# ariel415el/SoundEventDetection-Pytorch

Measured on AMD Instinct MI355X. Metric: SED train clips/sec (60s,64-mel,9-layer CNN), higher is better.
Workload: dtype bf16; 1 GPU; Cnn_AvgPooling main widths [32, 64, 128, 128], 60 s / 32 kHz / 64-mel clips (T=6001 frames, NFFT 1024, hop 320), batch 32/GPU, train step = waveform->log-mel->fwd->BCE->bwd->Adam-amsgrad; frontend_constants=bench, graph_replay=False, global_batch=32, frames=6001, parallelism=dp1, frontend_in_step=True, frontend_overlapped=False, frontend_overlap_mode=0, sync_bn=False, rccl_group=False, collectives_executed=False

## Files before the change

soundeventdetection-pytorch_amd/csrc/sed_conv_pc.hip:

```cpp
#include "conv_common.h"

#include <stdlib.h>


namespace {

#ifdef SED_STAMPS
constexpr bool kStamps = true;
#else
constexpr bool kStamps = false;
#endif

constexpr int kPcBlocks = 256;

__device__ __forceinline__ void wg_barrier() {
    asm volatile("s_waitcnt lgkmcnt(0)\n\ts_barrier" ::: "memory");
}

__device__ __forceinline__ int xswz(int col) { return (col >> 2) & 3; }
__device__ __forceinline__ f32x16 zero16() {
    f32x16 z;
#pragma unroll
    for (int i = 0; i < 16; ++i) z[i] = 0.f;
    return z;
}


template <typename T, int W, int WP, int TH, bool WRITE_MASK>
__device__ __forceinline__ void c1_build_tail(const C1Mma& c1m, const f32x16& d, T* __restrict__ xsb, int bi, int lane, int b, int h0, int H,
                                              unsigned short* __restrict__ maskg) {
    const int rr = bi >> 1, half = bi & 1, hh = lane >> 5;
    const int hr = h0 - 1 + rr;
    const int coll = half * 32 + (lane & 31) + 1;
    T* dst = xsb + (rr * WP + coll) * 32 + hh * 4;
    const int sw = (coll >> 2) & 3;
    if (hr < 0 || hr >= H) {
        asm volatile("" ::: "memory");
        float z4[4] = {0.f, 0.f, 0.f, 0.f};
#pragma unroll
        for (int g4 = 0; g4 < 4; ++g4) store4<T>(dst + ((g4 ^ sw) * 8), z4);
        return;
    }
    unsigned mk;
    const bool wm = WRITE_MASK && maskg != nullptr && (rr >= 2 || (rr == 1 && h0 == 0));
#if !defined(SED_C1_PKTAIL) || SED_C1_PKTAIL
    unsigned w[8];
    if (wm) c1mma_block_tail_pk<true>(d, w, mk);
    else c1mma_block_tail_pk<false>(d, w, mk);
#pragma unroll
    for (int g4 = 0; g4 < 4; ++g4) {
        u32x2 v2 = {w[2 * g4], w[2 * g4 + 1]};
        *reinterpret_cast<u32x2*>(dst + ((g4 ^ sw) * 8)) = v2;
    }
#else
    float a[16];
    if (wm) c1mma_block_tail<true>(c1m, d, a, mk);
    else c1mma_block_tail<false>(c1m, d, a, mk);
#pragma unroll
    for (int g4 = 0; g4 < 4; ++g4) {
// ... 19 lines not shown
#define DIV_TPI(n) ((n) / p.tilesPerImg)
#define DIV_NCH(n) ((n) / nchunks)
#endif
#ifndef SED_PC_ZEROC
#define SED_PC_ZEROC 0
#endif
#ifndef SED_PC_ONECH
#define SED_PC_ONECH 1
#endif
#ifndef SED_PC_WREGS
#define SED_PC_WREGS 1
#endif
#ifndef SED_PC_CSTAT
#define SED_PC_CSTAT 0
#endif
template <int W, int BN, int PRO, int EPI, bool COL = false, int NPW = 4, bool BLD = false, bool WR = false>
__global__ __launch_bounds__(256 + 64 * NPW + (BLD ? 256 : 0)) void conv_pc_kernel(ConvParams p) {
    typedef bf16_t T;
    constexpr int BM = 256, TH = BM / W, ROWS = TH + 2, WP = (W + 2 + 3) & ~3;
    constexpr int XS = ROWS * WP * 32;
    constexpr int WS = WR ? 0 : 9 * 32 * BN;
    constexpr int NT = BN / 32;
    constexpr int BNP = BN + 8;
    constexpr int OSZ = BM * BNP;
    constexpr int NP = 64 * NPW;
    constexpr int NTHR = 256 + NP + (BLD ? 256 : 0);
    static_assert(!WR || (!COL && !BLD && PRO != SED_PRO_C1 && EPI != SED_EPI_RELUBWD_C1 && (BN == 64 || BN == 128)), "WR: plain layers, 64 / 128-channel slices");
    static_assert(!(PRO == SED_PRO_DZBN || PRO == SED_PRO_DZPOOL) || (!COL && !BLD && TH % 2 == 0), "dz on load: even tile heights (pooled rows)");
    static_assert(!BLD || PRO == SED_PRO_C1, "builder waves: C1 mode, the four waves after the loader waves");
    constexpr int XITEMS = ROWS * W * 4, XIPT = (XITEMS + NP - 1) / NP;
    constexpr int WITEMS = WS / 8, WIPT = WR ? 1 : (WITEMS + NP - 1) / NP;
    constexpr int IPR = BN / 8, FIPT = BM * IPR / NP, FQS = NP / IPR;
    static_assert(W >= 8 && BM % W == 0 && (BM * IPR) % NP == 0 && NP % IPR == 0, "geometry");
    constexpr bool C1PRO = PRO == SED_PRO_C1;
    constexpr bool DZPRO = PRO == SED_PRO_DZBN || PRO == SED_PRO_DZPOOL;
    constexpr int NCOEF = DZPRO ? 5 : 2;
    constexpr bool C1EPI = EPI == SED_EPI_RELUBWD_C1;
    constexpr bool RELUBWD = EPI == SED_EPI_RELUBWD || C1EPI;
    constexpr bool PSTATS = EPI == SED_EPI_POOLSTATS;
    static_assert(!(C1PRO || C1EPI) || W == 64, "C1 mode: a thread's items are consecutive rows of one column (W = 64)");
    static_assert(!C1EPI || BN == 32, "C1 epilogue: the output channels are conv1's 32");
    static_assert(!C1EPI || NPW == 4, "C1 epilogue: item u of a loader thread is tile row u (FQS = W)");

    extern __shared__ __attribute__((aligned(16))) char smem[];
    const int H = p.H, Cinp = p.Cinp, Coutp = p.Coutp;
    const int nchunks = Cinp >> 5;
// ... 6 lines not shown
    float* pcoef = reinterpret_cast<float*>(os + nos * OSZ);
    constexpr int XTW = W + 2, XTR = ROWS + 2, XTN = XTR * XTW;
    typedef C1Tile<W, XTR> XTL;
    bf16_t* xt0 = reinterpret_cast<bf16_t*>(pcoef + NCOEF * Cinp);

    const int tid = threadIdx.x, lane = tid & 63, wave = tid >> 6;
    const int NY = Coutp / BN;
    const unsigned logical = xcd_remap(blockIdx.x, gridDim.x);
    const int by = logical % NY, bx = logical / NY, nbx = gridDim.x / NY;
    const int n0 = by * BN;
    const T* __restrict__ wg = reinterpret_cast<const T*>(p.wpack);
    const size_t wchunk_bytes = (size_t)36 * Coutp * 8 * 2;

    const int t_begin = bx * p.tpb;
    const int t_end = min(p.totalTiles, t_begin + p.tpb);
    const int nst = (t_end > t_begin ? t_end - t_begin : 0) * nchunks;
    const int NI = (nst + (WR ? 3 : 2) + 1) & ~1;

    {
        constexpr int NPAD = 2 * ROWS * 2 * 4;
        bf16x8 z8;
#pragma unroll
        for (int e = 0; e < 8; ++e) z8[e] = (bf16_t)0.f;
        for (int i = tid; i < NPAD; i += NTHR) {
            const int c16 = i & 3, side = (i >> 2) & 1, rowi = (i >> 3) % ROWS, sg = (i >> 3) / ROWS;
            *reinterpret_cast<bf16x8*>(xs0 + sg * XS + (rowi * WP + (side ? W + 1 : 0)) * 32 + c16 * 8) = z8;
        }
    }
    if (PRO == SED_PRO_BNRELU || C1PRO) {
        for (int i = tid; i < 2 * Cinp; i += NTHR) pcoef[i] = (i < Cinp ? p.pro_scale[i] : p.pro_shift[i - Cinp]);
    }
// ... 2 lines not shown
        for (int i = tid; i < 5 * Cinp; i += NTHR) {
            const int rowc = i / Cinp, c = i - rowc * Cinp;
            float v = 0.f;
            if (rowc == 0) v = p.dz_ca[c] * inv_pool;
            else if (rowc == 1) v = p.dz_cb[c];
            else if (rowc == 2) v = p.dz_cc[c];
            else if (PRO == SED_PRO_DZPOOL) v = rowc == 3 ? p.dz_sc[c] : p.dz_sh[c];
            pcoef[i] = v;
        }
    }
    if constexpr (C1PRO) {
        c1tile_init<W, XTR>(xt0, tid, NTHR);
        c1tile_init<W, XTR>(xt0 + XTL::N, tid, NTHR);
        __syncthreads();
        if (nst > 0) {
            const int b = DIV_TPI(t_begin), h0 = (t_begin - b * p.tilesPerImg) * TH;
            for (int e = tid; e < XTN; e += NTHR) {
                const int r = e / XTW, c = e - r * XTW;
                const int hy = h0 - 2 + r, wx = c - 1;
                float v = 0.f;
                if (hy >= 0 && hy < H && wx >= 0 && wx < W) {
                    v = p.c1_x[((size_t)b * H + hy) * W + wx];
                    if (p.c1_mean) v = (v - p.c1_mean[wx]) * (1.0f / p.c1_std[wx]);
                }
                c1tile_store<W, XTR>(xt0, r, c, v);
            }
        }
    }
    if constexpr (!WR) if (wres && nst > 0) {
        const int total = nchunks * WITEMS;
        for (int i = tid; i < total; i += NTHR) {
            const int c = i / WITEMS, it = i - c * WITEMS;
            const int rowi = it / BN, off = (it - rowi * BN) * 8;
            *reinterpret_cast<bf16x8*>(ws + c * WS + it * 8) =
                *reinterpret_cast<const bf16x8*>(wg + ((size_t)(c * 36 + rowi) * Coutp + n0) * 8 + off);
        }
    }
    __syncthreads();

    float S[8], Q[8];
#pragma unroll
    for (int e = 0; e < 8; ++e) { S[e] = 0.f; Q[e] = 0.f; }

    C1Mma c1m;
// ... 3 lines not shown
    if (C1PRO && (C1SHARE || wave < 4 || wave >= 4 + NPW)) {
        c1mma_init(c1m, p.c1_w, p.pro_scale, p.pro_shift, lane);
        if constexpr (C1PRO) {
            c1tile_lane_offsets<W, XTR>(0, lane, c1o[0][0], c1o[0][1]);
            c1tile_lane_offsets<W, XTR>(1, lane, c1o[1][0], c1o[1][1]);
        }
    }
    auto c1mfma = [&](int js, int rr, int half) -> f32x16 {
        const bf16_t* row = xt0 + (js & 1) * XTL::N + rr * XTL::XP;
        return half ? c1mma_block_mfma_b(c1m, row, c1o[1][0], c1o[1][1]) : c1mma_block_mfma_b(c1m, row, c1o[0][0], c1o[0][1]);
    };
    unsigned short* __restrict__ maskg = reinterpret_cast<unsigned short*>(p.c1_mask);
    auto build_c1 = [&](int js, int bw, auto part_c) __attribute__((always_inline)) {
        constexpr int PART = decltype(part_c)::value;
        if (js >= nst || (SED_DBG(p, 4))) return;
        const int tile = t_begin + js;
        const int b = DIV_TPI(tile), h0 = (tile - b * p.tilesPerImg) * TH;
        static_assert(!C1PRO || ((2 * TH) % 4 == 0), "whole blocks per wave");
        constexpr int NB = (2 * TH) / 4;
        T* img = xs0 + (js & 1) * XS;
        const bool reuse = js > 0 && h0 > 0;
        static_assert(!C1PRO || NB == 2, "part 1 / part 2 = fresh-row blocks 0 / 1 of a wave");
        constexpr int B0 = PART == 2 ? 1 : 0, B1 = PART == 1 ? 1 : (PART == 3 ? 0 : NB);
        constexpr bool TOP = PART != 2 && PART != 4;
        f32x16 dd[NB + 1];
#pragma unroll
        for (int blk = B0; blk < B1; ++blk)
            dd[blk] = c1mfma(js, 2 + ((bw + 4 * blk) >> 1), (bw + 4 * blk) & 1);
        if (TOP && !reuse) dd[NB] = c1mfma(js, bw >> 1, bw & 1);
#pragma unroll
        for (int blk = B0; blk < B1; ++blk)
            c1_build_tail<T, W, WP, TH, EPI == SED_EPI_STATS>(c1m, dd[blk], img, 4 + bw + 4 * blk, lane, b, h0, H, maskg);
        if constexpr (!TOP) return;
        if (!reuse) {
            c1_build_tail<T, W, WP, TH, EPI == SED_EPI_STATS>(c1m, dd[NB], img, bw, lane, b, h0, H, maskg);
        } else {
            const T* prev = xs0 + ((js - 1) & 1) * XS + TH * WP * 32;
            constexpr int NIT = 2 * WP * 32 / 8;
#pragma unroll
            for (int it = 0; it < (NIT + 255) / 256; ++it) {
                const int q = bw * 64 + lane + 256 * it;
                if (q < NIT) *reinterpret_cast<bf16x8*>(img + q * 8) = *reinterpret_cast<const bf16x8*>(prev + q * 8);
            }
        }
    };

    constexpr int C1NB = (2 * TH) / 4, C1NCP = (2 * WP * 32 / 8 + 255) / 256;
    f32x16 bdd[C1PRO ? C1NB + 1 : 1];
    bf16x8 bcp[C1PRO ? C1NCP : 1];
    auto build_c1_issue = [&](int js, int bw) __attribute__((always_inline)) {
        if (js >= nst) return;
        const int tile = t_begin + js;
        const int b = DIV_TPI(tile), h0 = (tile - b * p.tilesPerImg) * TH;
        const bool reuse = js > 0 && h0 > 0;
#pragma unroll
        for (int blk = 0; blk < C1NB; ++blk)
            bdd[blk] = c1mfma(js, 2 + ((bw + 4 * blk) >> 1), (bw + 4 * blk) & 1);
        if (!reuse) {
            bdd[C1NB] = c1mfma(js, bw >> 1, bw & 1);
        } else {
            const T* prev = xs0 + ((js - 1) & 1) * XS + TH * WP * 32;
            constexpr int NIT = 2 * WP * 32 / 8;
#pragma unroll
            for (int it = 0; it < C1NCP; ++it) {
                const int q = bw * 64 + lane + 256 * it;
                if (q < NIT) bcp[it] = *reinterpret_cast<const bf16x8*>(prev + q * 8);
            }
        }
    };
    auto build_c1_finish = [&](int js, int bw) __attribute__((always_inline)) {
        if (js >= nst) return;
        const int tile = t_begin + js;
        const int b = DIV_TPI(tile), h0 = (tile - b * p.tilesPerImg) * TH;
        T* img = xs0 + (js & 1) * XS;
        const bool reuse = js > 0 && h0 > 0;
#pragma unroll
        for (int blk = 0; blk < C1NB; ++blk)
            c1_build_tail<T, W, WP, TH, EPI == SED_EPI_STATS>(c1m, bdd[blk], img, 4 + bw + 4 * blk, lane, b, h0, H, maskg);
        if (!reuse) {
            c1_build_tail<T, W, WP, TH, EPI == SED_EPI_STATS>(c1m, bdd[C1NB], img, bw, lane, b, h0, H, maskg);
        } else {
            constexpr int NIT = 2 * WP * 32 / 8;
#pragma unroll
            for (int it = 0; it < C1NCP; ++it) {
                const int q = bw * 64 + lane + 256 * it;
                if (q < NIT) *reinterpret_cast<bf16x8*>(img + q * 8) = bcp[it];
            }
        }
    };
#if !defined(SED_C1_SPLITBUILD)
#define SED_C1_SPLITBUILD 0
#endif
    constexpr bool kSplitBuild = C1PRO && !BLD && SED_C1_SPLITBUILD;

    if (wave >= 4 && wave < 4 + NPW) {
// ... 10 lines not shown
        const int xrow0 = (pt >> 2) / W, xcol = (pt >> 2) % W + 1;
        const unsigned xvoff0 = (unsigned)(((xrow0 * W + xcol) * Cinp + cq * 8) * 2);
        const unsigned xvstep = (unsigned)(XRS * W * Cinp * 2);
        const int xlds0 = (xrow0 * WP + xcol) * 32 + ((cq ^ xswz(xcol)) * 8);
        constexpr bool XLASTFULL = (XITEMS % NP) == 0;
        const bool xlast_ok = XLASTFULL || (pt + (XIPT - 1) * NP) < XITEMS;
        auto xvoff = [&](int u2) -> unsigned { return (u2 == XIPT - 1 && !xlast_ok) ? SED_OOB : xvoff0 + (unsigned)u2 * xvstep; };
        auto xlds = [&](int u2) -> int { return xlds0 + u2 * XRS * WP * 32; };
        const unsigned wsrc0 = (unsigned)((((pt / BN) * Coutp + n0) * 8 + (pt % BN) * 8) * 2);
        const unsigned wstep = (unsigned)((NP / BN) * Coutp * 8 * 2);
        constexpr bool WLASTFULL = (WITEMS % NP) == 0;
        const bool wlast_ok = WLASTFULL || (pt + (WIPT - 1) * NP) < WITEMS;
        auto wsrc = [&](int u2) -> unsigned { return (u2 == WIPT - 1 && !wlast_ok) ? SED_OOB : wsrc0 + (unsigned)u2 * wstep; };
        const int fcg = pt % IPR, fq0 = pt / IPR;
        const unsigned fl_off0 = (unsigned)((fq0 * Coutp + n0 + fcg * 8) * 2);
        float ces[8], cet[8], cem[8];
        if (EPI == SED_EPI_RELUBWD) {
#pragma unroll
            for (int e = 0; e < 8; ++e) {
                ces[e] = p.epi_scale[n0 + fcg * 8 + e];
                cet[e] = p.epi_shift[n0 + fcg * 8 + e];
                cem[e] = p.epi_mean[n0 + fcg * 8 + e];
            }
        }

        constexpr int XTIPT = (XTN + NP - 1) / NP;
        struct XSet { Raw8<T> x[C1PRO ? 1 : XIPT]; float xr[C1PRO ? XTIPT : 1]; Raw8<T> g[DZPRO ? XIPT : 1]; };
        const int dz_psh = DZPRO ? (p.dz_pool >> 1) : 0;
        const int dz_Wo = W >> dz_psh;
        unsigned gvoff_[DZPRO ? XIPT : 1], svoff_[DZPRO ? XIPT : 1];
// ... 17 lines not shown
        if (C1PRO) {
#pragma unroll
            for (int u2 = 0; u2 < XTIPT; ++u2) {
                const int e = pt + u2 * NP, c = (e % XTW) - 1;
                const bool ok = e < XTN && c >= 0 && c < W;
                xtmu[u2] = (ok && p.c1_mean) ? p.c1_mean[c] : 0.f;
                xtis[u2] = ok ? (p.c1_std ? 1.0f / p.c1_std[c] : 1.0f) : 0.f;
            }
        }
        const size_t x1img_ = (size_t)H * W;

        auto stage_of = [&](int j, bool& live, int& b, int& h0, int& kc) {
            live = j >= 0 && j < nst;
            const int tl = live ? DIV_NCH(j) : 0;
            kc = live ? j - tl * nchunks : 0;
            const int tile = t_begin + tl;
            b = live ? DIV_TPI(tile) : 0;
            h0 = live ? (tile - b * p.tilesPerImg) * TH : 0;
        };
        auto issue_x = [&](XSet& r, int j) {
            bool live; int b, h0, kc;
            stage_of(j, live, b, h0, kc);
            live = live && !(SED_DBG(p, 8));
            if constexpr (C1PRO) {
                const size_t img = live ? x1img_ : 0;
                const __amdgpu_buffer_rsrc_t s1 = make_srd(p.c1_x + (size_t)b * img, img * 4);
#pragma unroll
                for (int u2 = 0; u2 < XTIPT; ++u2) {
                    const int e = pt + u2 * NP, rr = e / XTW, c = e - rr * XTW - 1;
                    const bool ok = e < XTN && c >= 0 && c < W;
                    r.xr[u2] = buf_load_f32(s1, ok ? (unsigned)(((h0 - 2 + rr) * W + c) * 4) : SED_OOB);
                }
                return;
// ... 7 lines not shown
                const T* __restrict__ gg = reinterpret_cast<const T*>(p.dz_g);
                if constexpr (PRO == SED_PRO_DZPOOL) {
                    const size_t pimg = live ? (size_t)(H >> dz_psh) * dz_Wo * Cinp : 0;
                    const __amdgpu_buffer_rsrc_t gsrd = make_srd(gg + (size_t)b * pimg, pimg * 2);
                    const unsigned gt = (unsigned)((((h0 >> dz_psh) * dz_Wo) * Cinp + kc * 32) * 2);
#pragma unroll
                    for (int u = 0; u < XIPT; ++u) r.g[u] = buf_load8<T>(gsrd, gvoff_[u] + gt);
                } else {
                    const __amdgpu_buffer_rsrc_t gsrd = make_srd(gg + (size_t)b * ximg, ximg * 2);
#pragma unroll
                    for (int u = 0; u < XIPT; ++u) r.g[u] = buf_load8<T>(gsrd, gvoff_[u] + xt);
                }
            }
        };
        auto issue_w = [&](int j) {
            if constexpr (WR) return;
            bool live; int b, h0, kc;
            stage_of(j, live, b, h0, kc);
            const size_t bytes = (live && !wres) ? wchunk_bytes * nchunks : 0;
            const __amdgpu_buffer_rsrc_t wsrd = make_srd(wg, bytes);
            const unsigned wo = (unsigned)(kc * wchunk_bytes);
#pragma unroll
            for (int u = 0; u < WIPT; ++u) wraw[u] = buf_load8<T>(wsrd, wsrc(u) + wo);
        };
        auto commit_w = [&](int j) {
            if constexpr (WR) return;
            if (wres || j >= nst) return;
            T* dst = ws + (j & 1) * WS;
#pragma unroll
            for (int u = 0; u < WIPT; ++u) {
                if (u == WIPT - 1 && pt + u * NP >= WITEMS) break;
                lds_store_raw<T>(dst + (pt + u * NP) * 8, wraw[u]);
            }
        };
        auto commit_x = [&](const XSet& r, int j, T* __restrict__ xsb) {
            bool live; int b, h0, kc;
            stage_of(j, live, b, h0, kc);
            if (j >= nst) return;
            if constexpr (C1PRO) return;
            if constexpr (DZPRO) {
                const int row_lo = h0 == 0 ? 1 : 0;
// ... 64 lines not shown
                if (!boundary) {
#pragma unroll
                    for (int u = 0; u < XIPT; ++u) {
                        if (u == XIPT - 1 && pt + u * NP >= XITEMS) break;
                        pro_item(u, false);
                    }
                } else {
#pragma unroll
                    for (int u = 0; u < XIPT; ++u) {
                        if (u == XIPT - 1 && pt + u * NP >= XITEMS) break;
                        pro_item(u, true);
                    }
                }
            }
        };
        auto tile_done_at = [&](int js, bool& yes, int& b, int& h0, int& par) {
            const int tl_ = DIV_NCH(js < 0 ? 0 : js);
            yes = js >= 0 && js < nst && (js - tl_ * nchunks) == nchunks - 1;
            const int tl = yes ? tl_ : 0;
            const int tile = t_begin + tl;
            b = yes ? DIV_TPI(tile) : 0;
            h0 = yes ? (tile - b * p.tilesPerImg) * TH : 0;
            par = tl & 1;
        };
        auto issue_z = [&](int j, auto ulo_c, auto uhi_c) {
            constexpr int ulo = decltype(ulo_c)::value, uhi = decltype(uhi_c)::value;
            if (!RELUBWD && !PSTATS) return;
            bool yes; int b, h0, par;
            tile_done_at(j - 1, yes, b, h0, par);
            if constexpr (C1EPI) {
                const size_t img = yes ? x1img_ : 0;
                const __amdgpu_buffer_rsrc_t s1 = make_srd(reinterpret_cast<const unsigned*>(p.c1_mask) + (size_t)b * img, img * 4);
#pragma unroll
                for (int u2 = 0; u2 < FIPT; ++u2)
                    mwd[u2] = __builtin_amdgcn_raw_buffer_load_b32(s1, (unsigned)(((h0 + u2) * W + fq0) * 4), 0, 0);
                return;
            }
// ... 6 lines not shown
                zraw[C1EPI ? 0 : u] = buf_load8<T>(rs, fl_off0 + (unsigned)(u * FQS * Coutp * 2) + tq);
            }
            if constexpr (PSTATS) {
                const __amdgpu_buffer_rsrc_t cs = make_srd(p.cnt + (size_t)b * zimg, zimg);
#pragma unroll
                for (int u = 0; u < FIPT; ++u)
                    if (u >= ulo && u < uhi) craw[u] = __builtin_bit_cast(u32x2, __builtin_amdgcn_raw_buffer_load_b64(cs, (fl_off0 + (unsigned)(u * FQS * Coutp * 2) + tq) >> 1, 0, 0));
            }
        };
        auto flush = [&](int j, auto ulo_c, auto uhi_c) {
            constexpr int ulo = decltype(ulo_c)::value, uhi = decltype(uhi_c)::value;
            bool yes; int b, h0, par;
            tile_done_at(j - 2, yes, b, h0, par);
            if (!yes || (SED_DBG(p, 32))) return;
            const T* osb = os + (nos == 2 ? par : 0) * OSZ;
            const __amdgpu_buffer_rsrc_t zs = make_srd(zg + (size_t)b * zimg_, zimg_ * 2);
            const unsigned tq = (unsigned)(h0 * W * Coutp * 2);
#pragma unroll
            for (int u = 0; u < FIPT; ++u) {
                if (u < ulo || u >= uhi) continue;
                const int q = fq0 + u * FQS;
                const bf16x8 raw = *reinterpret_cast<const bf16x8*>(osb + q * BNP + fcg * 8);
                const bool valid = h0 + q / W < H;
                if (RELUBWD) {
                    float v[8], z[8];
#pragma unroll
                    for (int e = 0; e < 8; ++e) v[e] = (float)raw[e];
                    if constexpr (C1EPI) {
#pragma unroll
                        for (int e = 0; e < 8; ++e) {
                            const bool on = (mwd[u] >> (16 * (e >> 2) + 4 * fcg + (e & 3))) & 1u;
                            const float gate = (valid && on) ? v[e] : 0.f;
                            v[e] = gate;
                            S[e] += gate;
                        }
                        if (!(SED_DBG(p, 1))) buf_store8<T>(zs, fl_off0 + (unsigned)(u * FQS * Coutp * 2) + tq, v);
                        continue;
                    } else {
// ... 187 lines not shown
                            for (int e = 0; e < 4; ++e) v[e] = acc[c][mt][4 * g + e];
                            store4<T>(osb + ostg0 + c * 32 + mt * 32 * BNP + 8 * g, v);
                        }
                if (kStamps) tc[2] += stamp() - c2;
            };
            for (int j = 0; j < NI; j += 2) {
                citer(std::integral_constant<int, 0>{}, j, xs0);
                citer(std::integral_constant<int, 1>{}, j + 1, xs0 + XS);
            }
            if (kStamps && (SED_DBG(p, 16)) && blockIdx.x == 8 && lane == 0 && wave == 1)
                printf("pc WR consumer wave %d: %d stages; cycles barrier %llu kloop %llu staging %llu total %llu\n", wave, NI, tc[0], tc[1], tc[2],
                       stamp() - t_start);
        } else {
        const int r = lane & 31, hh = lane >> 5;
        SED_SET_PRIO(p.dbg >> 10);
        int xoff[2][3][2], ostg[2];
#pragma unroll
        for (int mt = 0; mt < 2; ++mt) {
            const int q = (wave * 2 + mt) * 32 + r;
            const int prow = q / W, pcol = q % W;
            ostg[mt] = q * BNP + 4 * hh;
#pragma unroll
            for (int tj = 0; tj < 3; ++tj)
#pragma unroll
                for (int ks = 0; ks < 2; ++ks)
                    xoff[mt][tj][ks] = (prow * WP + pcol) * 32 + (((ks * 2 + hh) ^ xswz(pcol + tj)) * 8);
        }
        const int woff = (hh * BN + r) * 8;

        f32x16 acc[2][NT];
        f32x16 gacc, sacc;
        int offS[2] = {0, 0};
        if constexpr (CSTAT) {
#pragma unroll
            for (int i = 0; i < 16; ++i) { gacc[i] = 0.f; sacc[i] = 0.f; }
            const int i16 = lane & 15, gbit = (lane >> 4) & 1;
            const int qq = i16 >> 2, pp = i16 & 3;
#pragma unroll
            for (int half = 0; half < 2; ++half) offS[half] = (8 * hh + qq + 4 * half) * BNP + 16 * gbit + 4 * pp;
        }
        constexpr bool WREGS = C1PRO && NT == 1 && !COL && SED_PC_WREGS;
        bf16x8 wreg[WREGS ? 18 : 1];
        if constexpr (WREGS) {
            const T* __restrict__ wgl = reinterpret_cast<const T*>(p.wpack);
#pragma unroll
            for (int k = 0; k < 18; ++k) {
                const int tap = k >> 1, ks = k & 1;
                wreg[k] = *reinterpret_cast<const bf16x8*>(wgl + ((size_t)(tap * 4 + ks * 2 + hh) * Coutp + n0 + r) * 8);
            }
        }
        auto compute = [&](const T* __restrict__ xsb, const T* __restrict__ wsc, bool first) {
            if (SED_DBG(p, 2)) return;
            if constexpr (WREGS) {
                bf16x8 xf[3][2];
                auto ldx = [&](int k, bf16x8 (&xd)[2]) {
                    const int tap = k >> 1, ks = k & 1, ti = tap / 3, tj = tap % 3;
#pragma unroll
                    for (int mt = 0; mt < 2; ++mt)
                        xd[mt] = *reinterpret_cast<const bf16x8*>(xsb + xoff[mt][tj][ks] + (ti * WP + tj) * 32);
                };
                ldx(0, xf[0]);
                ldx(1, xf[1]);
#pragma unroll
                for (int k = 0; k < 18; ++k) {
                    if (k + 2 < 18) ldx(k + 2, xf[(k + 2) % 3]);
                    __builtin_amdgcn_sched_barrier(0);
#pragma unroll
                    for (int mt = 0; mt < 2; ++mt) acc[mt][0] = mfma(wreg[k], xf[k % 3][mt], acc[mt][0]);
                    __builtin_amdgcn_sched_barrier(0);
                }
                return;
            }
            constexpr int RD = 3;
            bf16x8 xf[RD][2], wf[RD][NT];
            auto ld = [&](int k, bf16x8 (&xd)[2], bf16x8 (&wd)[NT]) {
                const int tap = k >> 1, ks = k & 1, ti = tap / 3, tj = tap % 3;
#pragma unroll
                for (int mt = 0; mt < 2; ++mt)
                    xd[mt] = *reinterpret_cast<const bf16x8*>(xsb + xoff[mt][tj][ks] + (ti * WP + tj) * 32);
#pragma unroll
                for (int nt = 0; nt < NT; ++nt)
                    wd[nt] = *reinterpret_cast<const bf16x8*>(wsc + woff + ((tap * 4 + ks * 2) * BN + nt * 32) * 8);
            };
            constexpr int NK = COL ? 6 : 18;
            auto kmap = [](int s2) { return COL ? (s2 >> 1) * 6 + 2 + (s2 & 1) : s2; };
#pragma unroll
            for (int k = 0; k < RD - 1 && k < NK; ++k) ld(kmap(k), xf[k], wf[k]);
#pragma unroll
            for (int k = 0; k < NK; ++k) {
                if (k + RD - 1 < NK) ld(kmap(k + RD - 1), xf[(k + RD - 1) % RD], wf[(k + RD - 1) % RD]);
                __builtin_amdgcn_sched_barrier(0);
#pragma unroll
                for (int nt = 0; nt < NT; ++nt)
#pragma unroll
// ... 13 lines not shown

        unsigned long long tc[4] = {0, 0, 0, 0};
        auto stamp = [&]() -> unsigned long long { return kStamps ? __builtin_amdgcn_s_memtime() : 0ull; };
        auto citer = [&](int j, const T* __restrict__ xsb) {
            const unsigned long long c0 = stamp();
            wg_barrier();
            const unsigned long long c1 = stamp();
            tc[0] += c1 - c0;
            if (C1PRO && j >= nst) return;
            if (j >= nst) return;
            if constexpr (kSplitBuild) build_c1_issue(j + 1, wave);
            constexpr bool ONECH = C1PRO && SED_PC_ONECH;
            const int tl = ONECH ? j : DIV_NCH(j), kc = ONECH ? 0 : j - tl * nchunks;
            if (ONECH || (!SED_PC_ZEROC && kc == 0)) {
#pragma unroll
                for (int mt = 0; mt < 2; ++mt)
#pragma unroll
                    for (int nt = 0; nt < NT; ++nt)
#pragma unroll
                        for (int i = 0; i < 16; ++i) acc[mt][nt][i] = 0.f;
            }
            compute(xsb, ws + (wres ? kc : (j & 1)) * WS, kc == 0);
            const unsigned long long c2 = stamp();
            tc[1] += c2 - c1;
            if (!ONECH && kc != nchunks - 1) return;
            T* osb = os + (nos == 2 ? (tl & 1) : 0) * OSZ;
            if (!(SED_DBG(p, 128)))
#pragma unroll
            for (int mt = 0; mt < 2; ++mt)
#pragma unroll
                for (int nt = 0; nt < NT; ++nt)
#pragma unroll
                    for (int g = 0; g < 4; ++g) {
                        float v[4];
#pragma unroll
                        for (int e = 0; e < 4; ++e) v[e] = acc[mt][nt][4 * g + e];
                        store4<T>(osb + ostg[mt] + nt * 32 + 8 * g, v);
                    }
            const unsigned long long c3 = stamp();
            if constexpr (kSplitBuild) build_c1_finish(j + 1, wave);
            else if (C1PRO && !BLD) build_c1(j + 1, wave, std::integral_constant<int, C1SHARE ? (SED_C1_SHARE == 2 ? 3 : 1) : 0>{});
            if constexpr (CSTAT) {
                const int tile = t_begin + tl;
                const int b_ = DIV_TPI(tile), h0_ = (tile - b_ * p.tilesPerImg) * TH;
                bf16x8 ones;
#pragma unroll
                for (int e = 0; e < 8; ++e) ones[e] = (bf16_t)1.0f;
#pragma unroll
                for (int mt = 0; mt < 2; ++mt) {
                    const int q0s = (wave * 2 + mt) * 32;
                    if (h0_ + q0s / W < H) {
#pragma unroll
// ... 62 lines not shown
                if (!stat) {
                    tot = 0.25f * sraw;
                } else if (sc != 0.f && !ill) {
                    tot = (tot - 0.25f * beta * sraw) * (is / sc);
                } else {
                    if (tot != 0.f || sraw != 0.f) atomicOr(p.flag, 1);
                    tot = 0.f;
                }
            }
            p.partial[((size_t)bx * 2 + stat) * Coutp + n0 + cn] = tot;
            for (int row = bx + nbx; row < p.nparts; row += nbx) p.partial[((size_t)row * 2 + stat) * Coutp + n0 + cn] = 0.f;
        }
    }
}

template <int W, int BN, int PRO, int EPI, bool COL = false, int NPW = 4, bool BLD = false, bool WR = false>
int launch_pc_n(ConvParams& p, hipStream_t st) {
    constexpr int BM = 256, TH = BM / W, ROWS = TH + 2, WP = (W + 2 + 3) & ~3;
    const int nchunks = p.Cinp / 32;
    const int nos = nchunks == 1 ? 2 : 1;
    auto lds_for = [&](int wbufs_) -> size_t {
        return ((size_t)2 * ROWS * WP * 32 + (size_t)(WR ? 0 : wbufs_) * 9 * 32 * BN + (size_t)nos * BM * (BN + 8)) * sizeof(bf16_t) +
               (size_t)((PRO == SED_PRO_DZBN || PRO == SED_PRO_DZPOOL) ? 5 : 2) * p.Cinp * sizeof(float) +
               (PRO == SED_PRO_C1 ? (size_t)2 * C1Tile<W, ROWS + 2>::N * sizeof(bf16_t) : 0);
    };
    p.wres = (WR || nchunks <= 2 || lds_for(nchunks) <= 160 * 1024) ? 1 : 0;
    const size_t lds = lds_for(p.wres ? nchunks : 2);
    if (lds > 160 * 1024) return -1;
    if (p.dry) return 0;
    if (int rc_ = sed_set_max_lds<&conv_pc_kernel<W, BN, PRO, EPI, COL, NPW, BLD, WR>>(lds)) return rc_;
    p.tilesPerImg = cdiv(p.H, TH);
    p.totalTiles = p.B * p.tilesPerImg;
    sed_fastdiv_make((unsigned)p.tilesPerImg, &p.tpi_M, &p.tpi_l);
    sed_fastdiv_make((unsigned)nchunks, &p.nch_M, &p.nch_l);
    const int ny = p.Coutp / BN;
    long long blocks = kPcBlocks;
    if (const char* e = sed_getenv("SED_CONV_BLOCKS")) blocks = atoll(e) > 0 ? atoll(e) : blocks;
    int nbx = (int)(blocks / ny);
    if (nbx > p.nparts) nbx = p.nparts;
    if (nbx > p.totalTiles) nbx = p.totalTiles;
    if (nbx < 1) nbx = 1;
    p.tpb = cdiv(p.totalTiles, nbx);
    conv_pc_kernel<W, BN, PRO, EPI, COL, NPW, BLD, WR><<<dim3(nbx * ny), dim3(256 + 64 * NPW + (BLD ? 256 : 0)), lds, st>>>(p);
    return 0;
}

template <int W, int BN, int PRO, int EPI, bool COL = false, bool WR = false>
int launch_pc(ConvParams& p, hipStream_t st) {
    if constexpr (WR) {
        return launch_pc_n<W, BN, PRO, EPI, COL, 4, false, true>(p, st);
    } else {
#ifdef SED_EXPERIMENTS
    if constexpr (PRO == SED_PRO_C1 && BN == 32) {
        const char* e = sed_getenv("SED_PC_BUILDERS");
        if (e && e[0] == '1') return launch_pc_n<W, BN, PRO, EPI, COL, 4, true>(p, st);
        if (e && e[0] == '2') return launch_pc_n<W, BN, PRO, EPI, COL, 8, true>(p, st);
        if (e && e[0] == '3') return launch_pc_n<W, BN, PRO, EPI, COL, 8, false>(p, st);
    }
// ... 21 lines not shown
    if constexpr (!COL && (W == 16 || W == 8) && BN >= 64) {
        if (p.pro == SED_PRO_DZBN && p.epi == SED_EPI_POOLSTATS) return launch_pc<W, BN, SED_PRO_DZBN, SED_EPI_POOLSTATS, COL, WR>(p, st);
        if (p.pro == SED_PRO_DZBN && p.epi == SED_EPI_STORE) return launch_pc<W, BN, SED_PRO_DZBN, SED_EPI_STORE, COL, WR>(p, st);
        if (p.pro == SED_PRO_DZPOOL && p.epi == SED_EPI_RELUBWD) return launch_pc<W, BN, SED_PRO_DZPOOL, SED_EPI_RELUBWD, COL, WR>(p, st);
    }
#endif
    return -1;
}

int dispatch_pc_c1(ConvParams& p, hipStream_t st) {
    if (p.pro == SED_PRO_C1 && p.Cinp == 32) {
        if (p.Coutp % 64 == 0) {
            if (p.epi == SED_EPI_STATS) return launch_pc<64, 64, SED_PRO_C1, SED_EPI_STATS>(p, st);
            if (p.epi == SED_EPI_STORE) return launch_pc<64, 64, SED_PRO_C1, SED_EPI_STORE>(p, st);
        } else {
            if (p.epi == SED_EPI_STATS) return launch_pc<64, 32, SED_PRO_C1, SED_EPI_STATS>(p, st);
            if (p.epi == SED_EPI_STORE) return launch_pc<64, 32, SED_PRO_C1, SED_EPI_STORE>(p, st);
        }
    }
    if (p.pro == SED_PRO_NONE && p.epi == SED_EPI_RELUBWD_C1 && p.Coutp == 32)
        return launch_pc<64, 32, SED_PRO_NONE, SED_EPI_RELUBWD_C1>(p, st);
    return -1;
}

template <int W>
int dispatch_pc_bn(ConvParams& p, hipStream_t st) {
    if constexpr (W <= 32) {
        const char* ew = sed_getenv("SED_PC_WR");
        if (!(ew && ew[0] == '0')) {
            if (p.Coutp % 128 == 0 && p.Cinp >= 96) return dispatch_pc_pe<W, 128, false, true>(p, st);
        }
    }
// ... 25 lines not shown
```

Baseline: 7803 clips/s.

## Use 512-pixel tiles for the conv1-fused 32-channel forward conv stage

Adds a BM=512 variant of the persistent conv kernel for the C1-prologue, 32-output-channel forward layer. Each tile now covers 8 rows, with image-boundary-aware tile mapping so tiles never straddle images. Weights stay in registers instead of LDS, and the output staging buffer drops its padding in favour of an XOR swizzle. The goal is to amortize halo rebuild, barriers and per-stage overhead over twice the pixels. In exchange the kernel holds more accumulator registers, and the new tile indexing and mask limits add correctness risk.

New measurement: 7875 clips/s, median of 6. No clear change (+0.9%).

```diff
diff --git a/soundeventdetection-pytorch_amd/csrc/sed_conv_pc.hip b/soundeventdetection-pytorch_amd/csrc/sed_conv_pc.hip
--- a/soundeventdetection-pytorch_amd/csrc/sed_conv_pc.hip
+++ b/soundeventdetection-pytorch_amd/csrc/sed_conv_pc.hip
@@ -18,6 +18,7 @@
 }
 
 __device__ __forceinline__ int xswz(int col) { return (col >> 2) & 3; }
+__device__ __forceinline__ int oswz(int q) { return (q >> 2) & 3; }
 __device__ __forceinline__ f32x16 zero16() {
     f32x16 z;
 #pragma unroll
@@ -26,9 +27,9 @@
 }
 
 
-template <typename T, int W, int WP, int TH, bool WRITE_MASK>
+template <typename T, int W, int WP, int TH, bool WRITE_MASK, bool LIM = false>
 __device__ __forceinline__ void c1_build_tail(const C1Mma& c1m, const f32x16& d, T* __restrict__ xsb, int bi, int lane, int b, int h0, int H,
-                                              unsigned short* __restrict__ maskg) {
+                                              unsigned short* __restrict__ maskg, int hmk = 0) {
     const int rr = bi >> 1, half = bi & 1, hh = lane >> 5;
     const int hr = h0 - 1 + rr;
     const int coll = half * 32 + (lane & 31) + 1;
@@ -42,7 +43,7 @@
         return;
     }
     unsigned mk;
-    const bool wm = WRITE_MASK && maskg != nullptr && (rr >= 2 || (rr == 1 && h0 == 0));
+    const bool wm = WRITE_MASK && maskg != nullptr && (rr >= 2 || (rr == 1 && h0 == 0)) && (!LIM || hr <= hmk);
 #if !defined(SED_C1_PKTAIL) || SED_C1_PKTAIL
     unsigned w[8];
     if (wm) c1mma_block_tail_pk<true>(d, w, mk);
@@ -92,14 +93,19 @@
 #ifndef SED_PC_CSTAT
 #define SED_PC_CSTAT 0
 #endif
-template <int W, int BN, int PRO, int EPI, bool COL = false, int NPW = 4, bool BLD = false, bool WR = false>
+template <int W, int BN, int PRO, int EPI, bool COL = false, int NPW = 4, bool BLD = false, bool WR = false, int BM = 256>
 __global__ __launch_bounds__(256 + 64 * NPW + (BLD ? 256 : 0)) void conv_pc_kernel(ConvParams p) {
     typedef bf16_t T;
-    constexpr int BM = 256, TH = BM / W, ROWS = TH + 2, WP = (W + 2 + 3) & ~3;
+    constexpr int TH = BM / W, ROWS = TH + 2, WP = (W + 2 + 3) & ~3;
+    constexpr bool BIG = BM == 512;
+    constexpr bool NOWLDS = WR || BIG;
+    constexpr int MT = BM / 128;
     constexpr int XS = ROWS * WP * 32;
-    constexpr int WS = WR ? 0 : 9 * 32 * BN;
+    constexpr int WS = NOWLDS ? 0 : 9 * 32 * BN;
     constexpr int NT = BN / 32;
-    constexpr int BNP = BN + 8;
+    constexpr int BNP = BIG ? BN : BN + 8;
+    static_assert(BM == 256 || (BIG && W == 64 && BN == 32 && PRO == SED_PRO_C1 && !COL && !BLD && !WR && NPW == 4 && SED_PC_WREGS && !SED_PC_CSTAT &&
+                                (EPI == SED_EPI_STATS || EPI == SED_EPI_STORE)), "512-pixel stages: block 0's forward");
     constexpr int OSZ = BM * BNP;
     constexpr int NP = 64 * NPW;
     constexpr int NTHR = 256 + NP + (BLD ? 256 : 0);
@@ -107,7 +113,7 @@
     static_assert(!(PRO == SED_PRO_DZBN || PRO == SED_PRO_DZPOOL) || (!COL && !BLD && TH % 2 == 0), "dz on load: even tile heights (pooled rows)");
     static_assert(!BLD || PRO == SED_PRO_C1, "builder waves: C1 mode, the four waves after the loader waves");
     constexpr int XITEMS = ROWS * W * 4, XIPT = (XITEMS + NP - 1) / NP;
-    constexpr int WITEMS = WS / 8, WIPT = WR ? 1 : (WITEMS + NP - 1) / NP;
+    constexpr int WITEMS = WS / 8, WIPT = NOWLDS ? 1 : (WITEMS + NP - 1) / NP;
     constexpr int IPR = BN / 8, FIPT = BM * IPR / NP, FQS = NP / IPR;
     static_assert(W >= 8 && BM % W == 0 && (BM * IPR) % NP == 0 && NP % IPR == 0, "geometry");
     constexpr bool C1PRO = PRO == SED_PRO_C1;
@@ -144,7 +150,40 @@
 
     const int t_begin = bx * p.tpb;
     const int t_end = min(p.totalTiles, t_begin + p.tpb);
-    const int nst = (t_end > t_begin ? t_end - t_begin : 0) * nchunks;
+    const int tpi4 = (H + 3) >> 2;
+    int b0 = 0, i0 = 0, c0 = 0, T0 = 0, nst_big = 0;
+    if constexpr (BIG) {
+        const int ls = t_end > t_begin ? t_end - t_begin : 0;
+        b0 = t_begin / tpi4;
+        i0 = t_begin - b0 * tpi4;
+        c0 = tpi4 - i0;
+        T0 = (min(c0, ls) + 1) >> 1;
+        nst_big = T0;
+        if (ls > c0) {
+            const int rem = ls - c0, full = rem / tpi4;
+            nst_big += full * p.tilesPerImg + ((rem - full * tpi4 + 1) >> 1);
+        }
+    }
+    const int nst = BIG ? nst_big : (t_end > t_begin ? t_end - t_begin : 0) * nchunks;
+    auto tile_bh = [&](int tl, int& b, int& h0, int& hl) {
+        if constexpr (BIG) {
+            int i, g;
+            if (tl < T0) {
+                b = b0; i = i0 + 2 * tl; g = t_begin + 2 * tl;
+            } else {
+                const int t2 = tl - T0, q = DIV_TPI(t2);
+                b = b0 + 1 + q; i = 2 * (t2 - q * p.tilesPerImg); g = t_begin + c0 + q * tpi4 + i;
+            }
+            const int n = min(2, min(tpi4 - i, t_end - g));
+            h0 = 4 * i;
+            hl = min(H, h0 + 4 * n);
+        } else {
+            const int tile = t_begin + tl;
+            b = DIV_TPI(tile);
+            h0 = (tile - b * p.tilesPerImg) * TH;
+            hl = H;
+        }
+    };
     const int NI = (nst + (WR ? 3 : 2) + 1) & ~1;
 
     {
@@ -177,7 +216,8 @@
         c1tile_init<W, XTR>(xt0 + XTL::N, tid, NTHR);
         __syncthreads();
         if (nst > 0) {
-            const int b = DIV_TPI(t_begin), h0 = (t_begin - b * p.tilesPerImg) * TH;
+            int b, h0, hl_;
+            tile_bh(0, b, h0, hl_);
             for (int e = tid; e < XTN; e += NTHR) {
                 const int r = e / XTW, c = e - r * XTW;
                 const int hy = h0 - 2 + r, wx = c - 1;
@@ -190,7 +230,7 @@
             }
         }
     }
-    if constexpr (!WR) if (wres && nst > 0) {
+    if constexpr (!NOWLDS) if (wres && nst > 0) {
         const int total = nchunks * WITEMS;
         for (int i = tid; i < total; i += NTHR) {
             const int c = i / WITEMS, it = i - c * WITEMS;
@@ -224,14 +264,14 @@
     auto build_c1 = [&](int js, int bw, auto part_c) __attribute__((always_inline)) {
         constexpr int PART = decltype(part_c)::value;
         if (js >= nst || (SED_DBG(p, 4))) return;
-        const int tile = t_begin + js;
-        const int b = DIV_TPI(tile), h0 = (tile - b * p.tilesPerImg) * TH;
+        int b, h0, hl;
+        tile_bh(js, b, h0, hl);
         static_assert(!C1PRO || ((2 * TH) % 4 == 0), "whole blocks per wave");
         constexpr int NB = (2 * TH) / 4;
         T* img = xs0 + (js & 1) * XS;
         const bool reuse = js > 0 && h0 > 0;
-        static_assert(!C1PRO || NB == 2, "part 1 / part 2 = fresh-row blocks 0 / 1 of a wave");
-        constexpr int B0 = PART == 2 ? 1 : 0, B1 = PART == 1 ? 1 : (PART == 3 ? 0 : NB);
+        static_assert(!C1PRO || NB % 2 == 0, "part 1 / part 2 = the first / second half of a wave's fresh-row blocks");
+        constexpr int B0 = PART == 2 ? NB / 2 : 0, B1 = PART == 1 ? NB / 2 : (PART == 3 ? 0 : NB);
         constexpr bool TOP = PART != 2 && PART != 4;
         f32x16 dd[NB + 1];
 #pragma unroll
@@ -240,10 +280,10 @@
         if (TOP && !reuse) dd[NB] = c1mfma(js, bw >> 1, bw & 1);
 #pragma unroll
         for (int blk = B0; blk < B1; ++blk)
-            c1_build_tail<T, W, WP, TH, EPI == SED_EPI_STATS>(c1m, dd[blk], img, 4 + bw + 4 * blk, lane, b, h0, H, maskg);
+            c1_build_tail<T, W, WP, TH, EPI == SED_EPI_STATS, BIG>(c1m, dd[blk], img, 4 + bw + 4 * blk, lane, b, h0, H, maskg, hl);
         if constexpr (!TOP) return;
         if (!reuse) {
-            c1_build_tail<T, W, WP, TH, EPI == SED_EPI_STATS>(c1m, dd[NB], img, bw, lane, b, h0, H, maskg);
+            c1_build_tail<T, W, WP, TH, EPI == SED_EPI_STATS, BIG>(c1m, dd[NB], img, bw, lane, b, h0, H, maskg, hl);
         } else {
             const T* prev = xs0 + ((js - 1) & 1) * XS + TH * WP * 32;
             constexpr int NIT = 2 * WP * 32 / 8;
@@ -260,8 +300,8 @@
     bf16x8 bcp[C1PRO ? C1NCP : 1];
     auto build_c1_issue = [&](int js, int bw) __attribute__((always_inline)) {
         if (js >= nst) return;
-        const int tile = t_begin + js;
-        const int b = DIV_TPI(tile), h0 = (tile - b * p.tilesPerImg) * TH;
+        int b, h0, hl;
+        tile_bh(js, b, h0, hl);
         const bool reuse = js > 0 && h0 > 0;
 #pragma unroll
         for (int blk = 0; blk < C1NB; ++blk)
@@ -280,15 +320,15 @@
     };
     auto build_c1_finish = [&](int js, int bw) __attribute__((always_inline)) {
         if (js >= nst) return;
-        const int tile = t_begin + js;
-        const int b = DIV_TPI(tile), h0 = (tile - b * p.tilesPerImg) * TH;
+        int b, h0, hl;
+        tile_bh(js, b, h0, hl);
         T* img = xs0 + (js & 1) * XS;
         const bool reuse = js > 0 && h0 > 0;
 #pragma unroll
         for (int blk = 0; blk < C1NB; ++blk)
-            c1_build_tail<T, W, WP, TH, EPI == SED_EPI_STATS>(c1m, bdd[blk], img, 4 + bw + 4 * blk, lane, b, h0, H, maskg);
+            c1_build_tail<T, W, WP, TH, EPI == SED_EPI_STATS, BIG>(c1m, bdd[blk], img, 4 + bw + 4 * blk, lane, b, h0, H, maskg, hl);
         if (!reuse) {
-            c1_build_tail<T, W, WP, TH, EPI == SED_EPI_STATS>(c1m, bdd[C1NB], img, bw, lane, b, h0, H, maskg);
+            c1_build_tail<T, W, WP, TH, EPI == SED_EPI_STATS, BIG>(c1m, bdd[C1NB], img, bw, lane, b, h0, H, maskg, hl);
         } else {
             constexpr int NIT = 2 * WP * 32 / 8;
 #pragma unroll
@@ -329,6 +369,7 @@
         auto wsrc = [&](int u2) -> unsigned { return (u2 == WIPT - 1 && !wlast_ok) ? SED_OOB : wsrc0 + (unsigned)u2 * wstep; };
         const int fcg = pt % IPR, fq0 = pt / IPR;
         const unsigned fl_off0 = (unsigned)((fq0 * Coutp + n0 + fcg * 8) * 2);
+        const int fsl = (fcg ^ oswz(fq0)) * 8;
         float ces[8], cet[8], cem[8];
         if (EPI == SED_EPI_RELUBWD) {
 #pragma unroll
@@ -376,9 +417,10 @@
             live = j >= 0 && j < nst;
             const int tl = live ? DIV_NCH(j) : 0;
             kc = live ? j - tl * nchunks : 0;
-            const int tile = t_begin + tl;
-            b = live ? DIV_TPI(tile) : 0;
-            h0 = live ? (tile - b * p.tilesPerImg) * TH : 0;
+            int hl_;
+            tile_bh(tl, b, h0, hl_);
+            b = live ? b : 0;
+            h0 = live ? h0 : 0;
         };
         auto issue_x = [&](XSet& r, int j) {
             bool live; int b, h0, kc;
@@ -416,7 +458,7 @@
             }
         };
         auto issue_w = [&](int j) {
-            if constexpr (WR) return;
+            if constexpr (NOWLDS) return;
             bool live; int b, h0, kc;
             stage_of(j, live, b, h0, kc);
             const size_t bytes = (live && !wres) ? wchunk_bytes * nchunks : 0;
@@ -426,7 +468,7 @@
             for (int u = 0; u < WIPT; ++u) wraw[u] = buf_load8<T>(wsrd, wsrc(u) + wo);
         };
         auto commit_w = [&](int j) {
-            if constexpr (WR) return;
+            if constexpr (NOWLDS) return;
             if (wres || j >= nst) return;
             T* dst = ws + (j & 1) * WS;
 #pragma unroll
@@ -521,13 +563,14 @@
                 }
             }
         };
+        int fl_hl = 0;
         auto tile_done_at = [&](int js, bool& yes, int& b, int& h0, int& par) {
             const int tl_ = DIV_NCH(js < 0 ? 0 : js);
             yes = js >= 0 && js < nst && (js - tl_ * nchunks) == nchunks - 1;
             const int tl = yes ? tl_ : 0;
-            const int tile = t_begin + tl;
-            b = yes ? DIV_TPI(tile) : 0;
-            h0 = yes ? (tile - b * p.tilesPerImg) * TH : 0;
+            tile_bh(tl, b, h0, fl_hl);
+            b = yes ? b : 0;
+            h0 = yes ? h0 : 0;
             par = tl & 1;
         };
         auto issue_z = [&](int j, auto ulo_c, auto uhi_c) {
@@ -564,14 +607,14 @@
             tile_done_at(j - 2, yes, b, h0, par);
             if (!yes || (SED_DBG(p, 32))) return;
             const T* osb = os + (nos == 2 ? par : 0) * OSZ;
-            const __amdgpu_buffer_rsrc_t zs = make_srd(zg + (size_t)b * zimg_, zimg_ * 2);
+            const __amdgpu_buffer_rsrc_t zs = make_srd(zg + (size_t)b * zimg_, BIG ? (size_t)fl_hl * W * Coutp * 2 : zimg_ * 2);
             const unsigned tq = (unsigned)(h0 * W * Coutp * 2);
 #pragma unroll
             for (int u = 0; u < FIPT; ++u) {
                 if (u < ulo || u >= uhi) continue;
                 const int q = fq0 + u * FQS;
-                const bf16x8 raw = *reinterpret_cast<const bf16x8*>(osb + q * BNP + fcg * 8);
-                const bool valid = h0 + q / W < H;
+                const bf16x8 raw = *reinterpret_cast<const bf16x8*>(osb + q * BNP + (BIG ? fsl : fcg * 8));
+                const bool valid = h0 + q / W < (BIG ? fl_hl : H);
                 if (RELUBWD) {
                     float v[8], z[8];
 #pragma unroll
@@ -789,12 +832,14 @@
         } else {
         const int r = lane & 31, hh = lane >> 5;
         SED_SET_PRIO(p.dbg >> 10);
-        int xoff[2][3][2], ostg[2];
-#pragma unroll
-        for (int mt = 0; mt < 2; ++mt) {
-            const int q = (wave * 2 + mt) * 32 + r;
+        constexpr int MTO = BIG ? 1 : 2;
+        auto dmt = [](int mt) { return BIG ? (((mt * 32) / W) * WP + (mt * 32) % W) * 32 : 0; };
+        int xoff[MTO][3][2], ostg[MTO];
+#pragma unroll
+        for (int mt = 0; mt < MTO; ++mt) {
+            const int q = (wave * MT + mt) * 32 + r;
             const int prow = q / W, pcol = q % W;
-            ostg[mt] = q * BNP + 4 * hh;
+            ostg[mt] = q * BNP + 4 * hh + (BIG ? oswz(q) * 8 : 0);
 #pragma unroll
             for (int tj = 0; tj < 3; ++tj)
 #pragma unroll
@@ -803,7 +848,7 @@
         }
         const int woff = (hh * BN + r) * 8;
 
-        f32x16 acc[2][NT];
+        f32x16 acc[MT][NT];
         f32x16 gacc, sacc;
         int offS[2] = {0, 0};
         if constexpr (CSTAT) {
@@ -827,12 +872,12 @@
         auto compute = [&](const T* __restrict__ xsb, const T* __restrict__ wsc, bool first) {
             if (SED_DBG(p, 2)) return;
             if constexpr (WREGS) {
-                bf16x8 xf[3][2];
-                auto ldx = [&](int k, bf16x8 (&xd)[2]) {
+                bf16x8 xf[3][MT];
+                auto ldx = [&](int k, bf16x8 (&xd)[MT]) {
                     const int tap = k >> 1, ks = k & 1, ti = tap / 3, tj = tap % 3;
 #pragma unroll
-                    for (int mt = 0; mt < 2; ++mt)
-                        xd[mt] = *reinterpret_cast<const bf16x8*>(xsb + xoff[mt][tj][ks] + (ti * WP + tj) * 32);
+                    for (int mt = 0; mt < MT; ++mt)
+                        xd[mt] = *reinterpret_cast<const bf16x8*>(xsb + xoff[BIG ? 0 : mt][tj][ks] + (ti * WP + tj) * 32 + dmt(mt));
                 };
                 ldx(0, xf[0]);
                 ldx(1, xf[1]);
@@ -841,18 +886,19 @@
                     if (k + 2 < 18) ldx(k + 2, xf[(k + 2) % 3]);
                     __builtin_amdgcn_sched_barrier(0);
 #pragma unroll
-                    for (int mt = 0; mt < 2; ++mt) acc[mt][0] = mfma(wreg[k], xf[k % 3][mt], acc[mt][0]);
+                    for (int mt = 0; mt < MT; ++mt) acc[mt][0] = mfma(wreg[k], xf[k % 3][mt], acc[mt][0]);
                     __builtin_amdgcn_sched_barrier(0);
                 }
                 return;
             }
+            static_assert(WREGS || !BIG, "512-pixel stages: register-resident operator");
             constexpr int RD = 3;
             bf16x8 xf[RD][2], wf[RD][NT];
             auto ld = [&](int k, bf16x8 (&xd)[2], bf16x8 (&wd)[NT]) {
                 const int tap = k >> 1, ks = k & 1, ti = tap / 3, tj = tap % 3;
 #pragma unroll
                 for (int mt = 0; mt < 2; ++mt)
-                    xd[mt] = *reinterpret_cast<const bf16x8*>(xsb + xoff[mt][tj][ks] + (ti * WP + tj) * 32);
+                    xd[mt] = *reinterpret_cast<const bf16x8*>(xsb + xoff[BIG ? 0 : mt][tj][ks] + (ti * WP + tj) * 32);
 #pragma unroll
                 for (int nt = 0; nt < NT; ++nt)
                     wd[nt] = *reinterpret_cast<const bf16x8*>(wsc + woff + ((tap * 4 + ks * 2) * BN + nt * 32) * 8);
@@ -896,7 +942,7 @@
             const int tl = ONECH ? j : DIV_NCH(j), kc = ONECH ? 0 : j - tl * nchunks;
             if (ONECH || (!SED_PC_ZEROC && kc == 0)) {
 #pragma unroll
-                for (int mt = 0; mt < 2; ++mt)
+                for (int mt = 0; mt < MT; ++mt)
 #pragma unroll
                     for (int nt = 0; nt < NT; ++nt)
 #pragma unroll
@@ -909,7 +955,7 @@
             T* osb = os + (nos == 2 ? (tl & 1) : 0) * OSZ;
             if (!(SED_DBG(p, 128)))
 #pragma unroll
-            for (int mt = 0; mt < 2; ++mt)
+            for (int mt = 0; mt < MT; ++mt)
 #pragma unroll
                 for (int nt = 0; nt < NT; ++nt)
 #pragma unroll
@@ -917,7 +963,8 @@
                         float v[4];
 #pragma unroll
                         for (int e = 0; e < 4; ++e) v[e] = acc[mt][nt][4 * g + e];
-                        store4<T>(osb + ostg[mt] + nt * 32 + 8 * g, v);
+                        if constexpr (BIG) store4<T>(osb + (ostg[0] ^ (8 * g)) + mt * 32 * BNP, v);
+                        else store4<T>(osb + ostg[mt] + nt * 32 + 8 * g, v);
                     }
             const unsigned long long c3 = stamp();
             if constexpr (kSplitBuild) build_c1_finish(j + 1, wave);
@@ -1010,13 +1057,14 @@
     }
 }
 
-template <int W, int BN, int PRO, int EPI, bool COL = false, int NPW = 4, bool BLD = false, bool WR = false>
+template <int W, int BN, int PRO, int EPI, bool COL = false, int NPW = 4, bool BLD = false, bool WR = false, int BM = 256>
 int launch_pc_n(ConvParams& p, hipStream_t st) {
-    constexpr int BM = 256, TH = BM / W, ROWS = TH + 2, WP = (W + 2 + 3) & ~3;
+    constexpr int TH = BM / W, ROWS = TH + 2, WP = (W + 2 + 3) & ~3;
+    constexpr bool BIG = BM == 512;
     const int nchunks = p.Cinp / 32;
     const int nos = nchunks == 1 ? 2 : 1;
     auto lds_for = [&](int wbufs_) -> size_t {
-        return ((size_t)2 * ROWS * WP * 32 + (size_t)(WR ? 0 : wbufs_) * 9 * 32 * BN + (size_t)nos * BM * (BN + 8)) * sizeof(bf16_t) +
+        return ((size_t)2 * ROWS * WP * 32 + (size_t)((WR || BIG) ? 0 : wbufs_) * 9 * 32 * BN + (size_t)nos * BM * (BIG ? BN : BN + 8)) * sizeof(bf16_t) +
                (size_t)((PRO == SED_PRO_DZBN || PRO == SED_PRO_DZPOOL) ? 5 : 2) * p.Cinp * sizeof(float) +
                (PRO == SED_PRO_C1 ? (size_t)2 * C1Tile<W, ROWS + 2>::N * sizeof(bf16_t) : 0);
     };
@@ -1024,9 +1072,9 @@
     const size_t lds = lds_for(p.wres ? nchunks : 2);
     if (lds > 160 * 1024) return -1;
     if (p.dry) return 0;
-    if (int rc_ = sed_set_max_lds<&conv_pc_kernel<W, BN, PRO, EPI, COL, NPW, BLD, WR>>(lds)) return rc_;
-    p.tilesPerImg = cdiv(p.H, TH);
-    p.totalTiles = p.B * p.tilesPerImg;
+    if (int rc_ = sed_set_max_lds<&conv_pc_kernel<W, BN, PRO, EPI, COL, NPW, BLD, WR, BM>>(lds)) return rc_;
+    p.tilesPerImg = BIG ? cdiv(cdiv(p.H, 4), 2) : cdiv(p.H, TH);
+    p.totalTiles = BIG ? p.B * cdiv(p.H, 4) : p.B * p.tilesPerImg;
     sed_fastdiv_make((unsigned)p.tilesPerImg, &p.tpi_M, &p.tpi_l);
     sed_fastdiv_make((unsigned)nchunks, &p.nch_M, &p.nch_l);
     const int ny = p.Coutp / BN;
@@ -1037,7 +1085,7 @@
     if (nbx > p.totalTiles) nbx = p.totalTiles;
     if (nbx < 1) nbx = 1;
     p.tpb = cdiv(p.totalTiles, nbx);
-    conv_pc_kernel<W, BN, PRO, EPI, COL, NPW, BLD, WR><<<dim3(nbx * ny), dim3(256 + 64 * NPW + (BLD ? 256 : 0)), lds, st>>>(p);
+    conv_pc_kernel<W, BN, PRO, EPI, COL, NPW, BLD, WR, BM><<<dim3(nbx * ny), dim3(256 + 64 * NPW + (BLD ? 256 : 0)), lds, st>>>(p);
     return 0;
 }
 
@@ -1089,8 +1137,8 @@
             if (p.epi == SED_EPI_STATS) return launch_pc<64, 64, SED_PRO_C1, SED_EPI_STATS>(p, st);
             if (p.epi == SED_EPI_STORE) return launch_pc<64, 64, SED_PRO_C1, SED_EPI_STORE>(p, st);
         } else {
-            if (p.epi == SED_EPI_STATS) return launch_pc<64, 32, SED_PRO_C1, SED_EPI_STATS>(p, st);
-            if (p.epi == SED_EPI_STORE) return launch_pc<64, 32, SED_PRO_C1, SED_EPI_STORE>(p, st);
+            if (p.epi == SED_EPI_STATS) return launch_pc_n<64, 32, SED_PRO_C1, SED_EPI_STATS, false, 4, false, false, 512>(p, st);
+            if (p.epi == SED_EPI_STORE) return launch_pc_n<64, 32, SED_PRO_C1, SED_EPI_STORE, false, 4, false, false, 512>(p, st);
         }
     }
     if (p.pro == SED_PRO_NONE && p.epi == SED_EPI_RELUBWD_C1 && p.Coutp == 32)
```
